# panagiotou23/model-predictive-control

Measured on AMD Instinct MI355X. Metric: MPC solves/sec, bicycle model N=20 nx=4 nu=2, batch=65536; 1/2/4/8 GPU, higher is better.
Workload: dtype f64

## Files before the change

model_predictive_control_amd/csrc/mpc_api.hip:

```cpp
#include "../../include/mpc_hip.h"
#include "mpc_aux.hpp"
#include "mpc_solo.hpp"
#include "mpc_game.hpp"

#include <algorithm>
#include <chrono>
#include <cmath>
#include <cstdio>
#include <cstring>
#include <condition_variable>
#include <mutex>
#include <string>
#include <thread>
#include <array>
#include <vector>

using namespace mpc;

#define MPC_MAX_GROUPS 8
#define MPC_GRID_MAX_ROWS 1024

static thread_local std::string g_err;
static int fail(int code, const std::string &msg) { g_err = msg; return code; }

// ... 242 lines not shown
    int check = 0;
    num(getenv("MPC_CHECK_EVERY"), check);
    if (check > 0) h->check_every = check;
    h->spin = getenv("MPC_SPIN") != nullptr;
    h->host_timing = getenv("MPC_HOST_TIMING") != nullptr;
    if (const char *e = getenv("MPC_HOST_TRACE")) h->host_trace = e;
    const char *hwq = getenv("MPC_HW_QUEUES");
    h->hw_queues = hwq ? atoi(hwq) : probe_stream_concurrency(h);
}

extern "C" int mpc_create(const mpc_config *cfg, int device, mpc_handle **out)
{
    if (!cfg || !out) return fail(MPC_E_ARG, "mpc_create: null argument");
    {
        DevCfg probe;
        const int rcv = make_devcfg(*cfg, probe);
        if (rcv) return rcv;
    }
    int ndev = 0;
    HIPCHK(hipGetDeviceCount(&ndev));
    if (device < 0 || device >= ndev) return fail(MPC_E_ARG, "mpc_create: no such device");
    mpc_handle *h = new mpc_handle();
    h->solo_max = cfg->model == MPC_MODEL_PACEJKA ? 128 : 1024;
    h->solo_all = (cfg->model == MPC_MODEL_KINEMATIC && cfg->N <= 32) ? 4096 : 1024;
    h->cfg = *cfg;
    int rc = make_devcfg(*cfg, h->dc);
    if (rc) { delete h; return rc; }
    h->device = device;
    hipError_t e = hipSetDevice(device);
    if (e == hipSuccess) {
        int cus = 0;
        if (hipDeviceGetAttribute(&cus, hipDeviceAttributeMultiprocessorCount, device) == hipSuccess && cus > 0) h->num_cus = cus;
    }
    if (e == hipSuccess) e = hipHostMalloc((void **)&h->host_counts, 512, hipHostMallocDefault);
    if (e != hipSuccess) { delete h; return fail(MPC_E_HIP, std::string("mpc_create: ") + hipGetErrorString(e)); }
    read_switches(h);
    *out = h;
    return MPC_OK;
}

extern "C" int mpc_destroy(mpc_handle *h)
{
    if (!h) return MPC_OK;
    if (h->worker.joinable()) {
        { std::lock_guard<std::mutex> lk(h->mu); h->worker_quit = true; }
        h->cv.notify_all();
        h->worker.join();
    }
    (void)hipSetDevice(h->device);
    if (h->arena) (void)hipFree(h->arena);
    if (h->stage) (void)hipFree(h->stage);
    if (h->cl_gmeta) (void)hipFree(h->cl_gmeta);
    if (h->cl_gxy) (void)hipFree(h->cl_gxy);
    if (h->cl_gcells) (void)hipFree(h->cl_gcells);
    if (h->host_counts) (void)hipHostFree(h->host_counts);
    if (h->syncev) (void)hipEventDestroy(h->syncev);
    for (auto ev : h->ev_pool) (void)hipEventDestroy(ev);
    for (int g = 0; g < MPC_MAX_GROUPS; g++) if (h->gstream[g]) (void)hipStreamDestroy(h->gstream[g]);
    for (int g = 0; g <= MPC_MAX_GROUPS; g++) if (h->gevent[g]) (void)hipEventDestroy(h->gevent[g]);
    for (int b = 0; b < 2; b++) for (int g = 0; g < MPC_MAX_GROUPS; g++) if (h->pollev[b][g]) (void)hipEventDestroy(h->pollev[b][g]);
    for (int b = 0; b < 2; b++) for (int g = 0; g < MPC_MAX_GROUPS; g++) if (h->soloev[g][b]) (void)hipEventDestroy(h->soloev[g][b]);
    delete h;
    return MPC_OK;
}

static int reserve(mpc_handle *h, int B)
{
    const DevCfg &c = h->dc;
    const int Bp = (B + 63) & ~63;
    if (Bp <= h->Bp_alloc) { h->ws.Bp = h->Bp_alloc; h->ws.B = B; return MPC_OK; }
    HIPCHK(hipSetDevice(h->device));
    if (h->arena) { HIPCHK(hipFree(h->arena)); h->arena = nullptr; h->Bp_alloc = 0; }
    const size_t n = c.n, m = c.m ? c.m : 1, M = c.M, nx = c.nx, N = c.N;
    const size_t JS = nx * (nx + 1) + 2, St = 2 * (size_t)Bp + 64 * (MPC_MAX_GROUPS + 1);
    const size_t nd = 8 * n + 2 * M * n + 7 * m + REC;
    const size_t nscr = (N + 1) * nx + 2 * N + N + N * JS;
    const size_t ni = 4;
    const size_t bytes = (nd * 8 + ni * 4) * (size_t)Bp + nscr * 8 * St + 4 * St + 8 * 4 * MPC_MAX_GROUPS + 256 + 64 + 256;
    char *base = nullptr;
    hipError_t e = hipMalloc((void **)&base, bytes);
    if (e != hipSuccess) return fail(MPC_E_ALLOC, "workspace hipMalloc failed: " + std::string(hipGetErrorString(e)));
    h->arena = base; h->arena_bytes = bytes; h->Bp_alloc = Bp;
    Workspace &w = h->ws;
    double *dp = (double *)base;
    auto takeD = [&](size_t cnt) { double *r = dp; dp += cnt * (size_t)Bp; return r; };
    w.xk = takeD(n); w.gk = takeD(n); w.q = takeD(n); w.xn = takeD(n); w.xe = takeD(n); w.ge = takeD(n);
    w.xe2 = takeD(n); w.ge2 = takeD(n);
    w.S = takeD(M * n); w.Y = takeD(M * n);
    w.Sig = takeD(m); w.Sig_old = takeD(m); w.e1 = takeD(m); w.e2 = takeD(m);
    w.yhx = takeD(m); w.yhxn = takeD(m); w.yhe = takeD(m);
    w.rec = takeD(REC);
    auto takeS = [&](size_t cnt) { double *r = dp; dp += cnt * St; return r; };
    w.trajx = takeS((N + 1) * nx); w.useq = takeS(2 * N); w.stage_L = takeS(N); w.jac = takeS(N * JS);
    int *ip = (int *)dp;
    auto takeI = [&](size_t cnt) { int *r = ip; ip += cnt * (size_t)Bp; return r; };
    w.lists = takeI(4);
    w.agent_of = ip; ip += St;
    w.counts = ip;
    w.totals = (unsigned long long *)(ip + 8 * MPC_MAX_GROUPS);
    w.solo_ctr = (int *)(w.totals + 16);
    w.Bp = Bp; w.B = B; w.St = (int)St; w.Ls = Bp;
    w.ws_xe = w.xe; w.ws_ge = w.ge; w.ws_yhe = w.yhe; w.ws_Sig = w.Sig;
    HIPCHK(hipMemset(base, 0, bytes));
    return MPC_OK;
}

static int reserve_stage(mpc_handle *h, size_t bytes)
{
    if (bytes <= h->stage_bytes) return MPC_OK;
    if (h->stage) { HIPCHK(hipFree(h->stage)); h->stage = nullptr; h->stage_bytes = 0; }
    hipError_t e = hipMalloc((void **)&h->stage, bytes);
    if (e != hipSuccess) return fail(MPC_E_ALLOC, "staging hipMalloc failed");
    h->stage_bytes = bytes;
    return MPC_OK;
}

static inline dim3 grid_for(int B, int block) { return dim3((unsigned)((B + block - 1) / block)); }

template <int MODEL>
static bool launch_eval_t(mpc_handle *h, const Workspace &w, hipStream_t s, const int *lists, const int *counts,
                          int nG, int nC, hipEvent_t eva = nullptr, hipEvent_t evb = nullptr, int slot_bound = -1,
                          int *desc = nullptr)
{
    const DevCfg &c = h->dc;
    const bool shared = w.cl_index == nullptr;
    int nblk = counts ? 2 * (w.Bp / 64) : ((nG + 63) / 64 + (nC + 63) / 64);
    if (counts && slot_bound >= 0) nblk = std::min(nblk, (slot_bound + 126) / 64 + 1);
    if (nblk == 0) return true;
    const size_t lds = sizeof(double) * 64 * (size_t)(c.n + 1) + 64 * sizeof(int);
    bool wide = false;
    if constexpr (MODEL == KIN) {
        wide = counts && slot_bound >= 0 && slot_bound <= h->wide_max && c.nfe == 4 && c.N <= 64;
        if (wide)
            hipLaunchKernelGGL(rollout_wide_kernel, dim3((unsigned)(nblk * 16)), dim3(256), 0, s, c, w, lists, counts);
    }
    bool quad = false;
    if constexpr (MODEL == KIN) {
        quad = !wide && h->quad_rollout && c.nfe == 4 && c.N <= 64;
        if (quad)
            hipLaunchKernelGGL(rollout_pair_kernel, dim3((unsigned)(nblk * 2)), dim3(64),
                               sizeof(double) * 32 * (size_t)(c.n + 1), s, c, w, lists, counts, nG, nC);
    }
    if constexpr (MODEL == PAC) {
        quad = h->quad_rollout && !(counts && slot_bound >= 0 && slot_bound > h->pac_quad_max);
        if (quad)
            hipLaunchKernelGGL(rollout_quad_kernel, dim3((unsigned)(nblk * 4)), dim3(64),
                               sizeof(double) * 16 * (size_t)(c.n + 1), s, c, w, lists, counts, nG, nC);
    }
    if (!wide && !quad)
        hipLaunchKernelGGL((rollout_kernel<MODEL>), dim3((unsigned)nblk), dim3(64), lds, s, c, w, lists, counts, nG, nC);
    if (eva) (void)hipEventRecord(eva, s);
    if constexpr (MODEL == KIN) {
        if (h->fused_eval && (!counts || (slot_bound >= 0 && slot_bound <= h->fused_max))) {
            constexpr int JS = JacRec<MODEL>::SIZE;
            const int spb = FUSED_BLK / c.N;
            const int gb = (nblk * 64 + spb - 1) / spb;
            const size_t flds = sizeof(double) * (size_t)(JS + 1) * c.N * spb;
            if (shared)
                hipLaunchKernelGGL((stage_adjoint_kernel<MODEL, true>), dim3((unsigned)gb), dim3(FUSED_BLK), flds, s, c, w, counts, nG, nC, desc);
            else
                hipLaunchKernelGGL((stage_adjoint_kernel<MODEL, false>), dim3((unsigned)gb), dim3(FUSED_BLK), flds, s, c, w, counts, nG, nC, desc);
            if (evb) (void)hipEventRecord(evb, s);
            return true;
        }
    }
    const size_t xy_lds = (shared && w.near.gmeta && c.S <= GRID_LDS_MAX_S) ? sizeof(double) * 2 * (size_t)c.S : 0;
    if (shared)
        hipLaunchKernelGGL((stage_kernel<MODEL, true>), dim3((unsigned)(nblk * c.N)), dim3(64), xy_lds, s, c, w, counts, nG, nC, nblk);
    else
        hipLaunchKernelGGL((stage_kernel<MODEL, false>), dim3((unsigned)(nblk * c.N)), dim3(64), 0, s, c, w, counts, nG, nC, nblk);
    if (evb) (void)hipEventRecord(evb, s);
    hipLaunchKernelGGL((adjoint_kernel<MODEL>), dim3((unsigned)nblk), dim3(64), 0, s, c, w, counts, nG, nC, desc);
    return false;
}
static bool launch_eval(mpc_handle *h, const Workspace &w, hipStream_t s, const int *lists, const int *counts,
                        int nG, int nC, hipEvent_t eva = nullptr, hipEvent_t evb = nullptr, int slot_bound = -1,
                        int *desc = nullptr)
{
    if (h->dc.model == PAC) return launch_eval_t<PAC>(h, w, s, lists, counts, nG, nC, eva, evb, slot_bound, desc);
    return launch_eval_t<KIN>(h, w, s, lists, counts, nG, nC, eva, evb, slot_bound, desc);
}

static int refuse_if_busy(mpc_handle *h, const char *who)
{
    std::lock_guard<std::mutex> lk(h->mu);
    if (h->job_posted || h->job_running || h->job_done)
        return fail(MPC_E_ARG, std::string(who) + ": a solve of this handle is in flight (mpc_solve_wait first)");
    return MPC_OK;
}
static int check_common(mpc_handle *h, int B, const char *who, bool from_worker = false)
{
    if (!h) return fail(MPC_E_ARG, std::string(who) + ": null handle");
    if (B < 0) return fail(MPC_E_ARG, std::string(who) + ": negative batch");
    if (!from_worker) { const int rb = refuse_if_busy(h, who); if (rb) return rb; }
    HIPCHK(hipSetDevice(h->device));
    return MPC_OK;
}

static NearTab near_for(const mpc_handle *h, const double *cl)
{
    NearTab nt = {nullptr, nullptr, nullptr};
    if (h->nearest_mode == 2 && h->cl_grid_for && h->cl_grid_for == cl) { nt.gmeta = h->cl_gmeta; nt.gcells = h->cl_gcells; nt.gxy = h->cl_gxy; }
    return nt;
}

extern "C" int mpc_centerline_blocks(mpc_handle *h, const double *cl, int C, void *stream)
{
    int rc = check_common(h, C, "mpc_centerline_blocks"); if (rc) return rc;
    h->cl_grid_for = nullptr;
    if (C == 0 || !cl || C > MPC_GRID_MAX_ROWS) return MPC_OK;
    const DevCfg &c = h->dc;
    if (C > h->cl_grid_cap) {
        if (h->cl_gmeta) { HIPCHK(hipFree(h->cl_gmeta)); h->cl_gmeta = nullptr; }
        if (h->cl_gxy) { HIPCHK(hipFree(h->cl_gxy)); h->cl_gxy = nullptr; }
        if (h->cl_gcells) { HIPCHK(hipFree(h->cl_gcells)); h->cl_gcells = nullptr; }
        h->cl_grid_cap = 0;
        if (hipMalloc((void **)&h->cl_gmeta, sizeof(double) * GRID_META * (size_t)C) != hipSuccess ||
            hipMalloc((void **)&h->cl_gxy, sizeof(double) * 2 * (size_t)c.S * (size_t)C) != hipSuccess ||
            hipMalloc((void **)&h->cl_gcells, sizeof(unsigned) * (size_t)GRID_CELLS * (size_t)C) != hipSuccess)
            return fail(MPC_E_ALLOC, "centerline grid hipMalloc failed");
        h->cl_grid_cap = C;
    }
    hipStream_t s = (hipStream_t)stream;
    hipLaunchKernelGGL(cl_grid_meta_kernel, dim3((unsigned)C), dim3(64), 0, s, c, cl, C, h->cl_gmeta, h->cl_gxy);
    hipLaunchKernelGGL(cl_grid_cells_kernel, dim3(GRID_CELLS / 256, C), dim3(256), 0, s, c, cl, C, h->cl_gmeta, h->cl_gcells);
    HIPCHK(hipGetLastError());
    h->cl_grid_for = cl;
    return MPC_OK;
}

extern "C" int mpc_rhs(mpc_handle *h, int B, const double *x, const double *u, double *dx, void *stream)
{
    int rc = check_common(h, B, "mpc_rhs"); if (rc) return rc;
    if (B == 0) return MPC_OK;
    if (!x || !u || !dx) return fail(MPC_E_ARG, "mpc_rhs: null buffer");
    hipStream_t s = (hipStream_t)stream;
    if (h->dc.model == PAC) hipLaunchKernelGGL(rhs_kernel<PAC>, grid_for(B, 64), dim3(64), 0, s, h->dc, B, x, u, dx);
    else hipLaunchKernelGGL(rhs_kernel<KIN>, grid_for(B, 64), dim3(64), 0, s, h->dc, B, x, u, dx);
    HIPCHK(hipGetLastError());
    return MPC_OK;
}

extern "C" int mpc_rollout(mpc_handle *h, int B, int Nsim, const double *x0, const double *U, double *X,
                           void *stream)
{
    int rc = check_common(h, B, "mpc_rollout"); if (rc) return rc;
    if (B == 0 || Nsim == 0) return MPC_OK;
    if (Nsim < 0 || !x0 || !U || !X) return fail(MPC_E_ARG, "mpc_rollout: bad argument");
    hipStream_t s = (hipStream_t)stream;
    if (h->dc.model == PAC) hipLaunchKernelGGL(simulate_kernel<PAC>, grid_for(B, 64), dim3(64), 0, s, h->dc, B, Nsim, x0, U, X);
    else hipLaunchKernelGGL(simulate_kernel<KIN>, grid_for(B, 64), dim3(64), 0, s, h->dc, B, Nsim, x0, U, X);
    HIPCHK(hipGetLastError());
    return MPC_OK;
}

extern "C" int mpc_stage_errors(mpc_handle *h, int B, const double *pose, const double *cl,
                                const int32_t *cl_index, double *err, int32_t *idx, void *stream)
{
    int rc = check_common(h, B, "mpc_stage_errors"); if (rc) return rc;
    if (B == 0) return MPC_OK;
    if (!pose || !cl || !err) return fail(MPC_E_ARG, "mpc_stage_errors: null buffer");
    hipLaunchKernelGGL(errors_kernel, grid_for(B, 64), dim3(64), 0, (hipStream_t)stream, h->dc, B, pose, cl,
                       cl_index, near_for(h, cl), err, idx);
    HIPCHK(hipGetLastError());
    return MPC_OK;
}

extern "C" int mpc_lane_payoff(mpc_handle *h, int B, int K, const double *params15, const double *ego,
                               const double *cars, const int32_t *ncars, double *out, void *stream)
{
    int rc = check_common(h, B, "mpc_lane_payoff"); if (rc) return rc;
    if (B == 0) return MPC_OK;
    if (K < 0 || K > 62 || !params15 || !ego || (K > 0 && !cars) || !ncars || !out)
        return fail(MPC_E_ARG, "mpc_lane_payoff: bad argument");
    LaneParams p;
    std::memcpy(&p, params15, sizeof p);
    hipLaunchKernelGGL(lane_payoff_kernel, grid_for(B, 64), dim3(64), 0, (hipStream_t)stream, p, B, K, ego, cars,
                       ncars, out);
    HIPCHK(hipGetLastError());
    return MPC_OK;
}

extern "C" int mpc_math_probe(mpc_handle *h, int n, int op, const double *a, const double *b, double *out,
                              void *stream)
{
    int rc = check_common(h, n, "mpc_math_probe"); if (rc) return rc;
    if (n == 0) return MPC_OK;
    if (!a || !out || (op == 3 && !b)) return fail(MPC_E_ARG, "mpc_math_probe: null buffer");
    hipLaunchKernelGGL(math_probe_kernel, grid_for(n, 256), dim3(256), 0, (hipStream_t)stream, n, op, a, b, out);
    HIPCHK(hipGetLastError());
    return MPC_OK;
}

extern "C" int mpc_stage_cost(mpc_handle *h, int B, const double *x, const double *u, const double *cl,
                              const int32_t *cl_index, double *out, void *stream)
{
    int rc = check_common(h, B, "mpc_stage_cost"); if (rc) return rc;
    if (B == 0) return MPC_OK;
    if (!x || !u || !cl || !out) return fail(MPC_E_ARG, "mpc_stage_cost: null buffer");
    hipStream_t s = (hipStream_t)stream;
    if (h->dc.model == PAC) hipLaunchKernelGGL(stage_cost_kernel<PAC>, grid_for(B, 64), dim3(64), 0, s, h->dc, B, x, u, cl, cl_index, out);
    else hipLaunchKernelGGL(stage_cost_kernel<KIN>, grid_for(B, 64), dim3(64), 0, s, h->dc, B, x, u, cl, cl_index, out);
    HIPCHK(hipGetLastError());
    return MPC_OK;
}

static int eval_cost_grad(mpc_handle *h, int B, const double *x0, const double *cl, const int32_t *cl_index,
                          const double *U, const double *y, const double *Sigma, double *psi, double *grad,
                          double *yhat, void *stream, bool wave_path);
extern "C" int mpc_eval_cost_grad(mpc_handle *h, int B, const double *x0, const double *cl,
// ... 791 lines not shown
```

model_predictive_control_amd/csrc/mpc_eval.hpp:

```cpp
#pragma once
#include "mpc_solver.hpp"

#ifndef MPC_K1B_WAVES_PAC
#define MPC_K1B_WAVES_PAC 1
#endif
#ifndef MPC_QUAD_WAVES
#define MPC_QUAD_WAVES 2
#endif

namespace mpc {

struct SlotMap {
    int nG, nC, gpad, nblk_g, nblk;
    __device__ SlotMap(const int *counts, int nG_imm, int nC_imm)
    {
        nG = counts ? counts[0] : nG_imm;
        nC = counts ? counts[1] : nC_imm;
        gpad = (nG + 63) & ~63;
        nblk_g = gpad >> 6;
        nblk = nblk_g + ((nC + 63) >> 6);
    }
};

template <int MODEL>
__global__ void __launch_bounds__(64, 2)
rollout_kernel(const DevCfg c, const Workspace w, const int *__restrict__ lists,
               const int *__restrict__ counts, int nG_imm, int nC_imm)
{
    constexpr int NX = ModelDim<MODEL>::NX;
    extern __shared__ double lds[];
    double *tile = lds;
    int *s_agent = (int *)(lds + 64 * (c.n + 1));
    const SlotMap sm(counts, nG_imm, nC_imm);
    const int sb = blockIdx.x;
    if (sb >= sm.nblk) return;
    const int lane = threadIdx.x;
    const bool is_g = sb < sm.nblk_g;
    const int uslot = sb * 64 + lane;
    const int kslot = is_g ? uslot : uslot - sm.gpad;
    const bool active = kslot < (is_g ? sm.nG : sm.nC);
    const int *list = counts ? (is_g ? lists : lists + w.Ls) : nullptr;
    const int raw = active ? (list ? list[kslot] : kslot) : -1;
    const int a = raw < 0 ? -1 : raw & AGENT_MASK;
    const int n = c.n, N = c.N, ld = n + 1;
    s_agent[lane] = raw;
    w.agent_of[uslot] = raw;
    __syncthreads();
    const int total = 64 * n;
    for (int base = 0; base < total; base += 64 * 8) {
        double v[8];
        int off[8];
#pragma unroll
        for (int u = 0; u < 8; u++) {
            const int idx = base + u * 64 + lane;
            const int r = idx / n, j = idx - r * n;
            const int ar = idx < total ? s_agent[r] : -1;
            off[u] = ar >= 0 ? r * ld + j : -1;
            v[u] = ar >= 0 ? ((ar & CH2_BIT) ? w.xe2 : w.xe)[(size_t)(ar & AGENT_MASK) * n + j] : 0.0;
        }
#pragma unroll
        for (int u = 0; u < 8; u++) if (off[u] >= 0) tile[off[u]] = v[u];
    }
    __syncthreads();
    if (!active) return;
    const size_t St = (size_t)w.St;
    const double *urow = tile + lane * ld;
    double x[NX];
#pragma unroll
    for (int i = 0; i < NX; i++) { x[i] = w.x0[(size_t)a * NX + i]; w.trajx[(size_t)i * St + uslot] = x[i]; }
    for (int k = 0; k < N; k++) {
        const double d = urow[2 * k], dl = urow[2 * k + 1];
        w.useq[(size_t)(2 * k) * St + uslot] = d;
        w.useq[(size_t)(2 * k + 1) * St + uslot] = dl;
        StageInput<MODEL> u;
        prep_input(c, d, dl, u);
        stage_forward<MODEL>(c, u, x);
#pragma unroll
        for (int i = 0; i < NX; i++) w.trajx[(size_t)((k + 1) * NX + i) * St + uslot] = x[i];
    }
}

#ifndef MPC_K1A_WAVES
#define MPC_K1A_WAVES 3
#endif
template <class Put>
__device__ __forceinline__ void kin_wide_rollout(const DevCfg &c, const double (&x0)[4], double d, double dl, int lane, Put put);
__global__ void __launch_bounds__(64, MPC_K1A_WAVES)
rollout_pair_kernel(const DevCfg c, const Workspace w, const int *__restrict__ lists,
                    const int *__restrict__ counts, int nG_imm, int nC_imm)
{
#pragma clang fp contract(off)
#if MPC_DEV_STAMP == 1
    DevStamp stamp(blockIdx.x);
#endif
    constexpr int RPB = 32;
    extern __shared__ double lds[];
    const SlotMap sm(counts, nG_imm, nC_imm);
    const int lane = threadIdx.x, q = lane >> 1, half = lane & 1;
    const int uslot = blockIdx.x * RPB + q;
    const int nslots = sm.nblk * 64;
    const bool is_g = uslot < sm.gpad;
    const int kslot = is_g ? uslot : uslot - sm.gpad;
    const bool active = uslot < nslots && kslot < (is_g ? sm.nG : sm.nC);
    const int *list = counts ? (is_g ? lists : lists + w.Ls) : nullptr;
    const int raw = active ? (list ? list[kslot] : kslot) : -1;
    const int n = c.n, N = c.N, ld = n + 1;
    if (half == 0 && uslot < nslots) w.agent_of[uslot] = raw;
    if (__ballot(active) == 0ull) return;
    {
        const double *__restrict__ row = ((raw & CH2_BIT) ? w.xe2 : w.xe) + (size_t)(raw & AGENT_MASK) * n;
        for (int j0 = half; j0 < n; j0 += 16) {
            double v[8];
#pragma unroll
            for (int t = 0; t < 8; t++) v[t] = active && j0 + 2 * t < n ? row[j0 + 2 * t] : 0.0;
#pragma unroll
            for (int t = 0; t < 8; t++) if (j0 + 2 * t < n) lds[q * ld + j0 + 2 * t] = v[t];
        }
    }
    __builtin_amdgcn_wave_barrier();
    const int a = active ? raw & AGENT_MASK : 0;
    const size_t St = (size_t)w.St;
    const double *urow = lds + q * ld;
    double x[4];
#pragma unroll
    for (int i = 0; i < 4; i++) x[i] = active ? w.x0[(size_t)a * 4 + i] : 0.0;
    bool redo = false;
    auto put = [&](int k) {
        if (!active || redo) return;
        w.trajx[(size_t)(k * 4 + 2 * half) * St + uslot] = half ? x[2] : x[0];
        w.trajx[(size_t)(k * 4 + 2 * half + 1) * St + uslot] = half ? x[3] : x[1];
    };
    put(0);
    auto stage = [&](int k, const StageInput<KIN> &u) {
        const double d = urow[2 * k], dl = urow[2 * k + 1];
        if (active) w.useq[(size_t)(2 * k + half) * St + uslot] = half ? dl : d;
        redo = redo || !kin4_in_range(c, u, x);
#if MPC_DEV_STAMP == 1
        if (__ballot(redo) != 0ull) stamp.nfall++;
#endif
        double ph = x[2], v = x[3];
        KinRK k0, k1, k2, k3;
        const double ph0 = ph; kin_rk(c, u, v, k0); kin_next(c, k0, ph, v);
        const double ph1 = ph; kin_rk(c, u, v, k1); kin_next(c, k1, ph, v);
        const double ph2 = ph; kin_rk(c, u, v, k2); kin_next(c, k2, ph, v);
        const double ph3 = ph; kin_rk(c, u, v, k3); kin_next(c, k3, ph, v);
        KinRK ka, kb;
        ka.v1 = half ? k2.v1 : k0.v1; ka.v2 = half ? k2.v2 : k0.v2; ka.v3 = half ? k2.v3 : k0.v3; ka.v4 = half ? k2.v4 : k0.v4;
        ka.kp1 = half ? k2.kp1 : k0.kp1; ka.kp2 = half ? k2.kp2 : k0.kp2; ka.kp3 = half ? k2.kp3 : k0.kp3;
        kb.v1 = half ? k3.v1 : k1.v1; kb.v2 = half ? k3.v2 : k1.v2; kb.v3 = half ? k3.v3 : k1.v3; kb.v4 = half ? k3.v4 : k1.v4;
        kb.kp1 = half ? k3.kp1 : k1.kp1; kb.kp2 = half ? k3.kp2 : k1.kp2; kb.kp3 = half ? k3.kp3 : k1.kp3;
        double dxa, dya, dxb, dyb;
        kin_increment(c, u, half ? ph2 : ph0, ka, !redo, dxa, dya);
        kin_increment(c, u, half ? ph3 : ph1, kb, !redo, dxb, dyb);
        const double oxa = dpp_xchg<0xB1>(dxa), oya = dpp_xchg<0xB1>(dya);
        const double oxb = dpp_xchg<0xB1>(dxb), oyb = dpp_xchg<0xB1>(dyb);
        double px = x[0], py = x[1];
        px = px + dxa; py = py + dya;
        px = px + dxb; py = py + dyb;
        px = px + oxa; py = py + oya;
        px = px + oxb; py = py + oyb;
        x[0] = px; x[1] = py; x[2] = ph; x[3] = v;
        put(k + 1);
    };
    for (int k = 0; k < N; k += 2) {
        const int km = min(k + half, N - 1);
        StageInput<KIN> um, up;
#if MPC_DEV_STAMP == 1
        if (__ballot(!(fabs(urow[2 * km + 1]) <= 0.75)) != 0ull) stamp.nmid++;
        if (__ballot(!(fabs(urow[2 * km + 1]) < 1.0e5)) != 0ull) stamp.nslow++;
#endif
        prep_input(c, urow[2 * km], urow[2 * km + 1], um);
        up.ad = dpp_xchg<0xB1>(um.ad); up.beta = dpp_xchg<0xB1>(um.beta);
        up.sb_lr = dpp_xchg<0xB1>(um.sb_lr); up.cb_lr = dpp_xchg<0xB1>(um.cb_lr);
        up.dbeta = dpp_xchg<0xB1>(um.dbeta); up.mk0 = dpp_xchg<0xB1>(um.mk0); up.mk1 = dpp_xchg<0xB1>(um.mk1);
        StageInput<KIN> ua, ub;
        ua.ad = half ? up.ad : um.ad; ua.beta = half ? up.beta : um.beta; ua.sb_lr = half ? up.sb_lr : um.sb_lr;
        ua.cb_lr = half ? up.cb_lr : um.cb_lr; ua.dbeta = half ? up.dbeta : um.dbeta;
        ua.mk0 = half ? up.mk0 : um.mk0; ua.mk1 = half ? up.mk1 : um.mk1;
        ub.ad = half ? um.ad : up.ad; ub.beta = half ? um.beta : up.beta; ub.sb_lr = half ? um.sb_lr : up.sb_lr;
        ub.cb_lr = half ? um.cb_lr : up.cb_lr; ub.dbeta = half ? um.dbeta : up.dbeta;
        ub.mk0 = half ? um.mk0 : up.mk0; ub.mk1 = half ? um.mk1 : up.mk1;
        stage(k, ua);
        if (k + 1 < N) stage(k + 1, ub);
    }
    unsigned long long todo = __ballot(redo && active && half == 0);
    while (todo != 0ull) {
        const int l0 = (int)__builtin_ctzll(todo);
        todo &= todo - 1ull;
        const int aq = __builtin_amdgcn_readlane(raw, l0) & AGENT_MASK;
        const int uq = blockIdx.x * RPB + (l0 >> 1);
        const double *uro = lds + (l0 >> 1) * ld;
        const bool stage_lane = lane < N;
        const double dq = stage_lane ? uro[2 * lane] : 0.0, dlq = stage_lane ? uro[2 * lane + 1] : 0.0;
        double xq[4];
#pragma unroll
        for (int i = 0; i < 4; i++) xq[i] = w.x0[(size_t)aq * 4 + i];
        double *const tj = w.trajx + uq;
        kin_wide_rollout(c, xq, dq, dlq, lane, [=](int k, int i, double v) { tj[(size_t)(k * 4 + i) * St] = v; });
    }
}


__global__ void __launch_bounds__(64, MPC_QUAD_WAVES)
rollout_quad_kernel(const DevCfg c, const Workspace w, const int *__restrict__ lists,
                    const int *__restrict__ counts, int nG_imm, int nC_imm)
{
    constexpr int NX = 6, RPB = 16;
    extern __shared__ double lds[];
#if MPC_DEV_STAMP == 4
    DevStamp stamp(blockIdx.x);
#endif
    const SlotMap sm(counts, nG_imm, nC_imm);
    const int lane = threadIdx.x, q = lane >> 2, role = lane & 3;
    const int uslot = blockIdx.x * RPB + q;
    const int nslots = sm.nblk * 64;
    const bool is_g = uslot < sm.gpad;
    const int kslot = is_g ? uslot : uslot - sm.gpad;
    const bool active = uslot < nslots && kslot < (is_g ? sm.nG : sm.nC);
    const int *list = counts ? (is_g ? lists : lists + w.Ls) : nullptr;
    const int raw = active ? (list ? list[kslot] : kslot) : -1;
    const int n = c.n, N = c.N, ld = n + 1;
    if (role == 0 && uslot < nslots) w.agent_of[uslot] = raw;
    if (active) {
        const double *__restrict__ row = ((raw & CH2_BIT) ? w.xe2 : w.xe) + (size_t)(raw & AGENT_MASK) * n;
        for (int j0 = role; j0 < n; j0 += 32) {
            double v[8];
#pragma unroll
            for (int t = 0; t < 8; t++) v[t] = j0 + 4 * t < n ? row[j0 + 4 * t] : 0.0;
#pragma unroll
            for (int t = 0; t < 8; t++) if (j0 + 4 * t < n) lds[q * ld + j0 + 4 * t] = v[t];
        }
    }
    __builtin_amdgcn_wave_barrier();
    if (!active) return;
    const int a = raw & AGENT_MASK;
    const size_t St = (size_t)w.St;
    const double *urow = lds + q * ld;
    double x[NX];
#pragma unroll
    for (int i = 0; i < NX; i++) x[i] = w.x0[(size_t)a * NX + i];
    auto put = [&](int k) {
        w.trajx[(size_t)(k * NX + role) * St + uslot] = role == 0 ? x[0] : role == 1 ? x[1] : role == 2 ? x[2] : x[3];
        if (role < 2) w.trajx[(size_t)(k * NX + 4 + role) * St + uslot] = role == 0 ? x[4] : x[5];
    };
    put(0);
    for (int k = 0; k < N; k++) {
        const double d = urow[2 * k], dl = urow[2 * k + 1];
        if (role == 0) w.useq[(size_t)(2 * k) * St + uslot] = d;
        if (role == 1) w.useq[(size_t)(2 * k + 1) * St + uslot] = dl;
        StageInput<PAC> u;
        prep_input(c, d, dl, u);
#if MPC_DEV_STAMP == 4
        {
            bool fin = true;
#pragma unroll
            for (int i = 0; i < NX; i++) fin = fin && fabs(x[i]) < 1.0e300;
            const bool inr = fabs(x[2]) < 1.0e5 && fabs(dl) < 1.0e5 && (x[3] != 0.0 || (x[5] * c.lf + x[4] != 0.0 && x[5] * c.lr - x[4] != 0.0));
            if (__ballot(!fin) != 0ull) stamp.nfall++;
            if (__ballot(fin && !inr) != 0ull) stamp.nmid++;
            if (__ballot(!fin) != 0ull && k == 0) stamp.nslow++;
        }
#endif
        stage_forward_quad(c, u, x, role);
        put(k + 1);
    }
}

template <class Put>
__device__ __forceinline__ void kin_wide_rollout(const DevCfg &c, const double (&x0)[4], double d, double dl, int lane, Put put)
{
    const int N = c.N;
    const bool stage_lane = lane < N;
    StageInput<KIN> u;
    prep_input(c, d, dl, u);
    if (lane == 0) {
#pragma unroll
        for (int i = 0; i < 4; i++) put(0, i, x0[i]);
    }
    double ph = x0[2], v = x0[3];
    constexpr int PASS = 4;
    double cph[PASS] = {0.0, 0.0, 0.0, 0.0}, cv[PASS] = {0.0, 0.0, 0.0, 0.0}, eph = 0.0, ev = 0.0;
    int gen = 0;
    bool anygen = false;
#pragma unroll
    for (int p = 0; p < PASS; p++) {
        const int k1 = N < 16 * (p + 1) ? N : 16 * (p + 1);
        for (int k = 16 * p; k < k1; k++) {
            StageInput<KIN> uk;
            uk.ad = rdlane(u.ad, k); uk.beta = rdlane(u.beta, k); uk.sb_lr = rdlane(u.sb_lr, k);
            const double xs[4] = {0.0, 0.0, ph, v};
            const bool inr = __ballot(!kin4_in_range(c, uk, xs)) == 0ull;
            anygen = anygen || !inr;
#pragma unroll
            for (int j = 0; j < 4; j++) {
                if (lane == ((4 * k + j) & 63)) { cph[p] = ph; cv[p] = v; gen |= inr ? 0 : 1 << p; }
                KinRK kr;
                if (inr) { kin_rk(c, uk, v, kr); kin_next(c, kr, ph, v); }
                else { kin_gen_rk(c, uk, v, kr); kin_gen_next(c, kr, ph, v); }
            }
            if (lane == k) { eph = ph; ev = v; }
        }
    }
    double dx[PASS] = {0.0, 0.0, 0.0, 0.0}, dy[PASS] = {0.0, 0.0, 0.0, 0.0};
#pragma unroll
    for (int p = 0; p < PASS; p++) {
        const int s = 64 * p + lane;
        if (64 * p >= 4 * N) break;
        const int k = (s >> 2) < N ? (s >> 2) : N - 1;
        StageInput<KIN> uk;
        uk.ad = __shfl(u.ad, k); uk.beta = __shfl(u.beta, k); uk.sb_lr = __shfl(u.sb_lr, k);
        const bool g = ((gen >> p) & 1) != 0 && (s >> 2) < N;
        KinRK kr;
        kin_rk(c, uk, cv[p], kr);
        kin_increment(c, uk, cph[p], kr, !g, dx[p], dy[p]);
        if (anygen) {
            double gx, gy;
            kin_gen_rk(c, uk, g ? cv[p] : 0.0, kr);
            kin_gen_increment(c, uk, g ? cph[p] : 0.0, g ? cv[p] : 0.0, kr, gx, gy);
            dx[p] = g ? gx : dx[p]; dy[p] = g ? gy : dy[p];
        }
    }
    double px = x0[0], py = x0[1], epx = 0.0, epy = 0.0;
#pragma unroll
    for (int p = 0; p < PASS; p++) {
        const int k0 = 16 * p, k1 = N < 16 * (p + 1) ? N : 16 * (p + 1);
        for (int k = k0; k < k1; k++) {
#pragma clang fp contract(off)
#pragma unroll
            for (int j = 0; j < 4; j++) {
                px = px + rdlane(dx[p], (4 * k + j) & 63);
                py = py + rdlane(dy[p], (4 * k + j) & 63);
            }
            if (lane == k) { epx = px; epy = py; }
        }
    }
    if (stage_lane) { put(lane + 1, 0, epx); put(lane + 1, 1, epy); put(lane + 1, 2, eph); put(lane + 1, 3, ev); }
}

__global__ void __launch_bounds__(256)
rollout_wide_kernel(const DevCfg c, const Workspace w, const int *__restrict__ lists,
                    const int *__restrict__ counts)
{
    const SlotMap sm(counts, 0, 0);
    const int lane = threadIdx.x & 63, wv = threadIdx.x >> 6;
    const int uslot = blockIdx.x * 4 + wv;
    if (uslot >= sm.nblk * 64) return;
    const bool is_g = uslot < sm.gpad;
    const int kslot = is_g ? uslot : uslot - sm.gpad;
    const bool active = kslot < (is_g ? sm.nG : sm.nC);
    const int raw = active ? (is_g ? lists : lists + w.Ls)[kslot] : -1;
    if (lane == 0) w.agent_of[uslot] = raw;
    if (!active) return;
    const int a = raw & AGENT_MASK;
    const int N = c.N, n = c.n;
    const size_t St = (size_t)w.St;
    const double *__restrict__ row = ((raw & CH2_BIT) ? w.xe2 : w.xe) + (size_t)a * n;
    const bool stage_lane = lane < N;
    const double d = stage_lane ? row[2 * lane] : 0.0, dl = stage_lane ? row[2 * lane + 1] : 0.0;
    if (stage_lane) {
        w.useq[(size_t)(2 * lane) * St + uslot] = d;
        w.useq[(size_t)(2 * lane + 1) * St + uslot] = dl;
    }
    double x0[4];
#pragma unroll
    for (int i = 0; i < 4; i++) x0[i] = w.x0[(size_t)a * 4 + i];
    double *const tj = w.trajx + uslot;
    kin_wide_rollout(c, x0, d, dl, lane,
                     [=](int k, int i, double v) { tj[(size_t)(k * 4 + i) * St] = v; });
}

template <int MODEL> struct JacRec { static constexpr int SIZE = ModelDim<MODEL>::NX * (ModelDim<MODEL>::NX + 1) + 2; };

__device__ __forceinline__ void stage_geom(const DevCfg &c, const Workspace &w, const double *__restrict__ clp, int row,
                                           double px, double py, Geom &g)
{
    load_geom(c, clp, nearest_lookup(c, clp, w.near, row, px, py), g);
}

template <int MODEL, class Put>
__device__ __forceinline__ void stage_record(const DevCfg &c, const Workspace &w, int a, bool ch2, bool is_g,
                                             int k, const double (&xs)[ModelDim<MODEL>::NX],
                                             const double (&xe)[ModelDim<MODEL>::NX], double d, double dl,
                                             const Geom &g, Put put)
{
    constexpr int NX = ModelDim<MODEL>::NX, JS = JacRec<MODEL>::SIZE;
    double xb[NX], ub[2] = {0.0, 0.0};
#pragma unroll
    for (int i = 0; i < NX; i++) xb[i] = 0.0;
    double L = is_g ? stage_cost<MODEL, true>(c, g, xe, d, dl, xb, ub)
                    : stage_cost<MODEL, false>(c, g, xe, d, dl, xb, ub);
    if (c.sm) {
#pragma clang fp contract(off)
        const size_t am = (size_t)a * c.m;
#pragma unroll
        for (int i = 0; i < NX; i++) {
            if (i < c.sm) {
                const size_t kk = am + (size_t)(k * c.sm + i);
                const double gv = stage_constraint<MODEL>(c, g, xe, i);
                double lb, ubd;
                constraint_bounds(c, i, lb, ubd);
                const double sg = w.Sig[kk];
                const double zeta = gv + w.y[kk] / sg;
                const double zhat = fmax(lb, fmin(zeta, ubd));
                const double dd = zeta - zhat;
                const double yh = sg * dd;
                L = fma(0.5 * dd, yh, L);
                if (!ch2) w.yhe[kk] = yh;
                if (is_g) stage_constraint_adjoint<MODEL>(c, g, xe, i, yh, xb);
            }
        }
    }
    put(JS, L);
    if (is_g) {
#pragma unroll
        for (int i = 0; i < NX; i++) put(i, xb[i]);
        put(NX, ub[0]);
        put(NX + 1, ub[1]);
    }
}

template <int MODEL> __device__ __forceinline__ constexpr bool sens_is_const(int dd, int i)
{
    return (dd == 0 && i >= 2) || (MODEL == KIN && dd == 3 && i == 3);
}
__device__ __forceinline__ constexpr double sens_const(int dd, int i) { return dd == 0 && i == 2 ? 1.0 : 0.0; }

template <int MODEL, class Put>
__device__ __forceinline__ void stage_sens_record(const DevCfg &c, const double (&xs)[ModelDim<MODEL>::NX],
                                                  const double (&xe)[ModelDim<MODEL>::NX], double d, double dl, Put put)
{
    constexpr int NX = ModelDim<MODEL>::NX;
    StageInput<MODEL> u;
    prep_input(c, d, dl, u);
    double T[NX][NX];
    if constexpr (MODEL == PAC) {
        const bool lost = pac_stage_is_lost(u, xs);
        double xp[NX];
#pragma unroll
        for (int i = 0; i < NX; i++) xp[i] = xs[i];
        if (lost) pac_park(u, xp);
        stage_tangents_at<MODEL>(c, u, xp, xe, T);
#pragma unroll
        for (int dd = 0; dd < NX; dd++) {
#pragma unroll
            for (int i = 0; i < NX; i++)
                if (!sens_is_const<MODEL>(dd, i)) put(NX + 2 + dd * NX + i, lost ? __builtin_nan("") : T[dd][i]);
        }
        return;
    }
    stage_tangents_at<MODEL>(c, u, xs, xe, T);
#pragma unroll
    for (int dd = 0; dd < NX; dd++) {
#pragma unroll
        for (int i = 0; i < NX; i++) if (!sens_is_const<MODEL>(dd, i)) put(NX + 2 + dd * NX + i, T[dd][i]);
    }
}

template <int MODEL, class Get>
__device__ __forceinline__ void adjoint_rec_to(const DevCfg &c, bool is_g, Get get, double *psi_out, double *grow)
{
    constexpr int NX = ModelDim<MODEL>::NX, NZ = NX - 2, JS = JacRec<MODEL>::SIZE;
    const int N = c.N;
    double psi = 0.0;
    for (int k = 0; k < N; k++) psi += get(k, JS);
    if (psi_out) *psi_out = psi;
    if (!is_g) return;
    double lam[NX];
#pragma unroll
    for (int i = 0; i < NX; i++) lam[i] = 0.0;
    for (int k = N - 1; k >= 0; k--) {
#pragma unroll
        for (int i = 0; i < NX; i++) lam[i] += get(k, i);
        double gu[2], lz[NZ];
#pragma unroll
        for (int jj = 0; jj < 2; jj++) {
            double acc = get(k, NX + jj);
#pragma unroll
            for (int i = 0; i < NX; i++)
                acc = fma(sens_is_const<MODEL>(NZ + jj, i) ? sens_const(NZ + jj, i) : get(k, NX + 2 + (NZ + jj) * NX + i), lam[i], acc);
            gu[jj] = acc;
        }
#pragma unroll
        for (int jj = 0; jj < NZ; jj++) {
            double acc = 0.0;
#pragma unroll
            for (int i = 0; i < NX; i++)
                acc = fma(sens_is_const<MODEL>(jj, i) ? sens_const(jj, i) : get(k, NX + 2 + jj * NX + i), lam[i], acc);
            lz[jj] = acc;
        }
#pragma unroll
        for (int jj = 0; jj < NZ; jj++) lam[2 + jj] = lz[jj];
        grow[2 * k] = gu[0];
        grow[2 * k + 1] = gu[1];
    }
}
template <int MODEL, class Get>
__device__ __forceinline__ void adjoint_rec(const DevCfg &c, const Workspace &w, int a, bool ch2, bool is_g, Get get)
{
    double *psi_out = w.psi_direct ? w.psi_direct + a : !ch2 ? w.rec + (size_t)a * REC + R_PSIE : nullptr;
    adjoint_rec_to<MODEL>(c, is_g, get, psi_out, (ch2 ? w.ge2 : w.ge) + (size_t)a * c.n);
}

template <class Get>
__device__ __forceinline__ void adjoint_rec_quad_kin(const DevCfg &c, bool is_g, int comp, Get get, double *psi_out, double *grow)
{
    constexpr int NX = 4, NZ = 2, JS = JacRec<KIN>::SIZE;
    const int N = c.N;
    if (comp == 0) {
        double psi = 0.0;
        for (int k = 0; k < N; k++) psi += get(k, JS);
        if (psi_out) *psi_out = psi;
    }
    if (!is_g) return;
    const int dd = (comp + 2) & 3;
    double lam = 0.0;
    for (int k = N - 1; k >= 0; k--) {
        lam += get(k, comp);
        const double l0 = quad_bcast<0x00>(lam), l1 = quad_bcast<0x55>(lam), l2 = quad_bcast<0xAA>(lam), l3 = quad_bcast<0xFF>(lam);
        double acc = comp < 2 ? get(k, NX + comp) : 0.0;
        const double t0 = get(k, NX + 2 + dd * NX + 0), t1 = get(k, NX + 2 + dd * NX + 1);
        const double t2 = dd == 0 ? 1.0 : get(k, NX + 2 + dd * NX + 2);
        const double t3 = (dd == 0 || dd == 3) ? 0.0 : get(k, NX + 2 + dd * NX + 3);
        acc = fma(t0, l0, acc);
        acc = fma(t1, l1, acc);
        acc = fma(t2, l2, acc);
        acc = fma(t3, l3, acc);
        if (comp < 2) grow[2 * k + comp] = acc;
        else lam = acc;
    }
    static_assert(sens_is_const<KIN>(0, 2) && sens_is_const<KIN>(0, 3) && sens_is_const<KIN>(3, 3) && !sens_is_const<KIN>(3, 2) &&
                  !sens_is_const<KIN>(1, 3) && !sens_is_const<KIN>(2, 3) && !sens_is_const<KIN>(0, 1), "constant entries of the kinematic block");
    (void)NZ;
}

#ifndef MPC_K1B_WAVES
#define MPC_K1B_WAVES 3
#endif

template <int MODEL, bool SHARED_CL>
__global__ void __launch_bounds__(64, (MODEL == KIN ? MPC_K1B_WAVES : MPC_K1B_WAVES_PAC))
stage_kernel(const DevCfg c, const Workspace w, const int *__restrict__ counts, int nG_imm, int nC_imm,
             int nblk_max)
{
    constexpr int NX = ModelDim<MODEL>::NX, JS = JacRec<MODEL>::SIZE;
#if MPC_DEV_STAMP == 6
    DevStamp stamp(blockIdx.x);
#endif
    const SlotMap sm(counts, nG_imm, nC_imm);
    const int k = blockIdx.x / nblk_max, sb = blockIdx.x % nblk_max;
    if (sb >= sm.nblk) return;
    const bool is_g = sb < sm.nblk_g;
    const int uslot = sb * 64 + threadIdx.x;
    const int raw = w.agent_of[uslot];
    extern __shared__ double2 s_xy[];
    const bool lds_xy = SHARED_CL && w.near.gmeta != nullptr && c.S <= GRID_LDS_MAX_S;
    if (lds_xy) {
        const double2 *__restrict__ gp = reinterpret_cast<const double2 *>(w.near.gxy);
        for (int j = threadIdx.x; j < c.S; j += 64) s_xy[j] = gp[j];
        __builtin_amdgcn_wave_barrier();
    }
    if (raw < 0) return;
    const int a = raw & AGENT_MASK;
    const bool ch2 = (raw & CH2_BIT) != 0;
    const size_t St = (size_t)w.St;
    double xs[NX], xe[NX];
#pragma unroll
    for (int i = 0; i < NX; i++) {
        xs[i] = w.trajx[(size_t)(k * NX + i) * St + uslot];
        xe[i] = w.trajx[(size_t)((k + 1) * NX + i) * St + uslot];
    }
    const double d = w.useq[(size_t)(2 * k) * St + uslot], dl = w.useq[(size_t)(2 * k + 1) * St + uslot];
    const double *__restrict__ clp = SHARED_CL ? w.cl : w.cl + (size_t)w.cl_index[a] * 2 * (size_t)c.S;
    double *const jr = w.jac + (size_t)k * JS * St + uslot;
    double *const sl = w.stage_L + (size_t)k * St + uslot;
    const auto put = [=](int f, double v) { *(f == JS ? sl : jr + (size_t)f * St) = v; };
    if (is_g) stage_sens_record<MODEL>(c, xs, xe, d, dl, put);
    Geom g;
    if (lds_xy) {
        const int idx = nearest_index_grid(c, clp, w.near.gmeta, w.near.gcells, [=](int i) { return s_xy[i]; }, xe[0], xe[1]);
        load_geom_xy(s_xy, idx, g);
    } else {
        stage_geom(c, w, clp, SHARED_CL ? 0 : w.cl_index[a], xe[0], xe[1], g);
    }
    stage_record<MODEL>(c, w, a, ch2, is_g, k, xs, xe, d, dl, g, put);
}

template <int MODEL>
__global__ void __launch_bounds__(64)
adjoint_kernel(const DevCfg c, const Workspace w, const int *__restrict__ counts, int nG_imm, int nC_imm,
               int *__restrict__ desc)
{
    constexpr int JS = JacRec<MODEL>::SIZE;
    const SlotMap sm(counts, nG_imm, nC_imm);
    const int sb = blockIdx.x;
    if (desc && sb == 0 && threadIdx.x == 0) *desc = sm.gpad;
    if (sb >= sm.nblk) return;
    const bool is_g = sb < sm.nblk_g;
    const int uslot = sb * 64 + threadIdx.x;
    const int raw = w.agent_of[uslot];
    if (raw < 0) return;
    const size_t St = (size_t)w.St;
    const double *const jac = w.jac + uslot, *const sl = w.stage_L + uslot;
    adjoint_rec<MODEL>(c, w, raw & AGENT_MASK, (raw & CH2_BIT) != 0, is_g, [=](int k, int f) {
        return f == JS ? sl[(size_t)k * St] : jac[((size_t)k * JS + f) * St];
    });
}

constexpr int FUSED_BLK = 256;

#ifndef MPC_FUSED_WAVES
#define MPC_FUSED_WAVES 3
#endif
template <int MODEL, bool SHARED_CL>
__global__ void __launch_bounds__(FUSED_BLK, MPC_FUSED_WAVES)
stage_adjoint_kernel(const DevCfg c, const Workspace w, const int *__restrict__ counts, int nG_imm, int nC_imm,
                     int *__restrict__ desc)
{
    static_assert(MODEL == KIN, "the fused K1b + K1c kernel is the kinematic model's");
    constexpr int NX = ModelDim<MODEL>::NX, JS = JacRec<MODEL>::SIZE, BLK = FUSED_BLK;
    extern __shared__ double s_rec[];
#if MPC_DEV_STAMP == 2
    DevStamp stamp(blockIdx.x * (BLK / 64) + (threadIdx.x >> 6));
#endif
    const SlotMap sm(counts, nG_imm, nC_imm);
    const int N = c.N, SPB = BLK / N;
    const int slot0 = blockIdx.x * SPB, nslots = sm.nblk * 64;
    if (desc && blockIdx.x == 0 && threadIdx.x == 0) *desc = sm.gpad;
    if (slot0 >= nslots) return;
    const size_t St = (size_t)w.St;
    const int NS = N * SPB;
    {
        const int k = threadIdx.x / SPB, j = threadIdx.x - k * SPB;
        const int uslot = slot0 + j;
        const int raw = (k < N && uslot < nslots) ? w.agent_of[uslot] : -1;
        if (raw >= 0) {
            const bool is_g = uslot < sm.gpad;
            const int a = raw & AGENT_MASK;
            const bool ch2 = (raw & CH2_BIT) != 0;
            double xs[NX], xe[NX];
#pragma unroll
            for (int i = 0; i < NX; i++) {
                xs[i] = w.trajx[(size_t)(k * NX + i) * St + uslot];
                xe[i] = w.trajx[(size_t)((k + 1) * NX + i) * St + uslot];
            }
            const double d = w.useq[(size_t)(2 * k) * St + uslot], dl = w.useq[(size_t)(2 * k + 1) * St + uslot];
            const double *__restrict__ clp = SHARED_CL ? w.cl : w.cl + (size_t)w.cl_index[a] * 2 * (size_t)c.S;
            double *const r = s_rec + k * SPB + j;
            const auto put = [=](int f, double v) { r[(size_t)f * NS] = v; };
            if (is_g) stage_sens_record<MODEL>(c, xs, xe, d, dl, put);
            Geom g;
            stage_geom(c, w, clp, SHARED_CL ? 0 : w.cl_index[a], xe[0], xe[1], g);
            stage_record<MODEL>(c, w, a, ch2, is_g, k, xs, xe, d, dl, g, put);
        }
    }
    __syncthreads();
    for (int t = threadIdx.x; t < 4 * SPB; t += BLK) {
        const int j = t >> 2, comp = t & 3, uslot = slot0 + j;
        const int raw = uslot < nslots ? w.agent_of[uslot] : -1;
        if (raw < 0) continue;
        const double *const rj = s_rec + j;
        const int a = raw & AGENT_MASK;
        const bool ch2 = (raw & CH2_BIT) != 0;
        double *psi_out = w.psi_direct ? w.psi_direct + a : !ch2 ? w.rec + (size_t)a * REC + R_PSIE : nullptr;
        adjoint_rec_quad_kin(c, uslot < sm.gpad, comp, [=](int k, int f) { return rj[(size_t)f * NS + k * SPB]; },
                             psi_out, (ch2 ? w.ge2 : w.ge) + (size_t)a * c.n);
    }
}

}
```

Before: 501,400.

## Split kinematic sensitivity into hot/cold paths and compact fused LDS record

Adds a hot path for the kinematic stage sensitivities that uses the endpoint-aware RK4 tangent routine when inputs are in range. Out-of-range lanes fall back to a cold path that reloads the state and recomputes the tangents after a ballot. The fused stage-adjoint kernel's shared-memory record drops three constant rows through a row remap, which shrinks LDS per block. Kernel arguments are re-fetched through a KernArgs accessor inside scoped blocks, apparently to shorten register live ranges. The cost is more code and a divergent cold path, and the compact row mapping must stay in sync with the adjoint reader.

```diff
diff --git a/model_predictive_control_amd/csrc/mpc_api.hip b/model_predictive_control_amd/csrc/mpc_api.hip
--- a/model_predictive_control_amd/csrc/mpc_api.hip
+++ b/model_predictive_control_amd/csrc/mpc_api.hip
@@ -418,10 +418,10 @@
     if (eva) (void)hipEventRecord(eva, s);
     if constexpr (MODEL == KIN) {
         if (h->fused_eval && (!counts || (slot_bound >= 0 && slot_bound <= h->fused_max))) {
-            constexpr int JS = JacRec<MODEL>::SIZE;
-            const int spb = FUSED_BLK / c.N;
+            const FusedTile tile(c.N);
+            const int spb = tile.spb;
             const int gb = (nblk * 64 + spb - 1) / spb;
-            const size_t flds = sizeof(double) * (size_t)(JS + 1) * c.N * spb;
+            const size_t flds = tile.bytes();
             if (shared)
                 hipLaunchKernelGGL((stage_adjoint_kernel<MODEL, true>), dim3((unsigned)gb), dim3(FUSED_BLK), flds, s, c, w, counts, nG, nC, desc);
             else
diff --git a/model_predictive_control_amd/csrc/mpc_eval.hpp b/model_predictive_control_amd/csrc/mpc_eval.hpp
--- a/model_predictive_control_amd/csrc/mpc_eval.hpp
+++ b/model_predictive_control_amd/csrc/mpc_eval.hpp
@@ -86,10 +86,12 @@
 template <class Put>
 __device__ __forceinline__ void kin_wide_rollout(const DevCfg &c, const double (&x0)[4], double d, double dl, int lane, Put put);
 __global__ void __launch_bounds__(64, MPC_K1A_WAVES)
-rollout_pair_kernel(const DevCfg c, const Workspace w, const int *__restrict__ lists,
+rollout_pair_kernel(const DevCfg cfg, const Workspace ws, const int *__restrict__ lists,
                     const int *__restrict__ counts, int nG_imm, int nC_imm)
 {
 #pragma clang fp contract(off)
+    const DevCfg &c = cfg;
+    const Workspace &w = ws;
 #if MPC_DEV_STAMP == 1
     DevStamp stamp(blockIdx.x);
 #endif
@@ -119,21 +121,21 @@
     }
     __builtin_amdgcn_wave_barrier();
     const int a = active ? raw & AGENT_MASK : 0;
-    const size_t St = (size_t)w.St;
     const double *urow = lds + q * ld;
     double x[4];
 #pragma unroll
     for (int i = 0; i < 4; i++) x[i] = active ? w.x0[(size_t)a * 4 + i] : 0.0;
     bool redo = false;
-    auto put = [&](int k) {
+    auto put = [&](const Workspace &w, int k) {
         if (!active || redo) return;
+        const size_t St = (size_t)w.St;
         w.trajx[(size_t)(k * 4 + 2 * half) * St + uslot] = half ? x[2] : x[0];
         w.trajx[(size_t)(k * 4 + 2 * half + 1) * St + uslot] = half ? x[3] : x[1];
     };
-    put(0);
-    auto stage = [&](int k, const StageInput<KIN> &u) {
+    put(w, 0);
+    auto stage = [&](const DevCfg &c, const Workspace &w, int k, const StageInput<KIN> &u) {
         const double d = urow[2 * k], dl = urow[2 * k + 1];
-        if (active) w.useq[(size_t)(2 * k + half) * St + uslot] = half ? dl : d;
+        if (active) w.useq[(size_t)(2 * k + half) * (size_t)w.St + uslot] = half ? dl : d;
         redo = redo || !kin4_in_range(c, u, x);
 #if MPC_DEV_STAMP == 1
         if (__ballot(redo) != 0ull) stamp.nfall++;
@@ -160,9 +162,12 @@
         px = px + oxa; py = py + oya;
         px = px + oxb; py = py + oyb;
         x[0] = px; x[1] = py; x[2] = ph; x[3] = v;
-        put(k + 1);
+        put(w, k + 1);
     };
     for (int k = 0; k < N; k += 2) {
+        const KernArgs ka;
+        const DevCfg &c = ka.c();
+        const Workspace &w = ka.w();
         const int km = min(k + half, N - 1);
         StageInput<KIN> um, up;
 #if MPC_DEV_STAMP == 1
@@ -180,11 +185,15 @@
         ub.ad = half ? um.ad : up.ad; ub.beta = half ? um.beta : up.beta; ub.sb_lr = half ? um.sb_lr : up.sb_lr;
         ub.cb_lr = half ? um.cb_lr : up.cb_lr; ub.dbeta = half ? um.dbeta : up.dbeta;
         ub.mk0 = half ? um.mk0 : up.mk0; ub.mk1 = half ? um.mk1 : up.mk1;
-        stage(k, ua);
-        if (k + 1 < N) stage(k + 1, ub);
+        stage(c, w, k, ua);
+        if (k + 1 < N) stage(c, w, k + 1, ub);
     }
     unsigned long long todo = __ballot(redo && active && half == 0);
     while (todo != 0ull) {
+        const KernArgs ka;
+        const DevCfg &c = ka.c();
+        const Workspace &w = ka.w();
+        const size_t St = (size_t)w.St;
         const int l0 = (int)__builtin_ctzll(todo);
         todo &= todo - 1ull;
         const int aq = __builtin_amdgcn_readlane(raw, l0) & AGENT_MASK;
@@ -456,6 +465,41 @@
     }
 }
 
+template <class Put>
+__device__ __forceinline__ bool stage_sens_record_kin_hot(const DevCfg &c, const double (&xs)[4], const double (&xe)[4],
+                                                          double d, double dl, Put put)
+{
+    StageInput<KIN> u;
+    prep_input(c, d, dl, u);
+    const bool ok = c.nfe == 4 && kin4_in_range(c, u, xs);
+    const double xa[4] = {xs[0], xs[1], ok ? xs[2] : 0.0, ok ? xs[3] : 0.0};
+    double T[4][4];
+    stage_tangents_kin4(c, u, xa, xe, T);
+#pragma unroll
+    for (int dd = 0; dd < 4; dd++) {
+#pragma unroll
+        for (int i = 0; i < 4; i++) if (!sens_is_const<KIN>(dd, i)) put(6 + dd * 4 + i, T[dd][i]);
+    }
+    return !ok;
+}
+template <class Put>
+__device__ __forceinline__ void stage_sens_record_kin_cold(const DevCfg &c, const double *__restrict__ trajx,
+                                                           const double *__restrict__ useq, size_t St, Put put)
+{
+    double xs[4];
+#pragma unroll
+    for (int i = 0; i < 4; i++) xs[i] = trajx[(size_t)i * St];
+    StageInput<KIN> u;
+    prep_input(c, useq[0], useq[St], u);
+    double T[4][4];
+    stage_tangents<KIN>(c, u, xs, T);
+#pragma unroll
+    for (int dd = 0; dd < 4; dd++) {
+#pragma unroll
+        for (int i = 0; i < 4; i++) if (!sens_is_const<KIN>(dd, i)) put(6 + dd * 4 + i, T[dd][i]);
+    }
+}
+
 template <int MODEL, class Get>
 __device__ __forceinline__ void adjoint_rec_to(const DevCfg &c, bool is_g, Get get, double *psi_out, double *grow)
 {
@@ -574,7 +618,11 @@
     double *const jr = w.jac + (size_t)k * JS * St + uslot;
     double *const sl = w.stage_L + (size_t)k * St + uslot;
     const auto put = [=](int f, double v) { *(f == JS ? sl : jr + (size_t)f * St) = v; };
-    if (is_g) stage_sens_record<MODEL>(c, xs, xe, d, dl, put);
+    bool cold = false;
+    if (is_g) {
+        if constexpr (MODEL == KIN) cold = stage_sens_record_kin_hot(c, xs, xe, d, dl, put);
+        else stage_sens_record<MODEL>(c, xs, xe, d, dl, put);
+    }
     Geom g;
     if (lds_xy) {
         const int idx = nearest_index_grid(c, clp, w.near.gmeta, w.near.gcells, [=](int i) { return s_xy[i]; }, xe[0], xe[1]);
@@ -583,6 +631,14 @@
         stage_geom(c, w, clp, SHARED_CL ? 0 : w.cl_index[a], xe[0], xe[1], g);
     }
     stage_record<MODEL>(c, w, a, ch2, is_g, k, xs, xe, d, dl, g, put);
+    if constexpr (MODEL == KIN) {
+        if (__builtin_expect(__ballot(cold) != 0ull, 0)) {
+            const KernArgs ka;
+            const Workspace &wc = ka.w();
+            const size_t Sc = (size_t)wc.St;
+            if (cold) stage_sens_record_kin_cold(ka.c(), wc.trajx + (size_t)(k * NX) * Sc + uslot, wc.useq + (size_t)(2 * k) * Sc + uslot, Sc, put);
+        }
+    }
 }
 
 template <int MODEL>
@@ -607,13 +663,22 @@
 }
 
 constexpr int FUSED_BLK = 256;
+struct FusedTile {
+    static constexpr int ROWS = JacRec<KIN>::SIZE + 1 - 3;
+    int spb, ns;
+    __host__ __device__ explicit FusedTile(int N) : spb(FUSED_BLK / N), ns(N * (FUSED_BLK / N)) {}
+    __host__ __device__ size_t bytes() const { return sizeof(double) * (size_t)ROWS * ns; }
+    __host__ __device__ static constexpr int row(int f) { return f == JacRec<KIN>::SIZE ? ROWS - 1 : f >= 6 + 4 ? f - 2 : f; }
+};
+static_assert(FusedTile::row(6 + 1) == 7 && FusedTile::row(6 + 4) == 8 && FusedTile::row(6 + 14) == 18 &&
+              FusedTile::row(JacRec<KIN>::SIZE) == 19 && FusedTile::ROWS == 20, "the rows of the kinematic record");
 
 #ifndef MPC_FUSED_WAVES
 #define MPC_FUSED_WAVES 3
 #endif
 template <int MODEL, bool SHARED_CL>
 __global__ void __launch_bounds__(FUSED_BLK, MPC_FUSED_WAVES)
-stage_adjoint_kernel(const DevCfg c, const Workspace w, const int *__restrict__ counts, int nG_imm, int nC_imm,
+stage_adjoint_kernel(const DevCfg cfg, const Workspace ws, const int *__restrict__ counts, int nG_imm, int nC_imm,
                      int *__restrict__ desc)
 {
     static_assert(MODEL == KIN, "the fused K1b + K1c kernel is the kinematic model's");
@@ -622,38 +687,69 @@
 #if MPC_DEV_STAMP == 2
     DevStamp stamp(blockIdx.x * (BLK / 64) + (threadIdx.x >> 6));
 #endif
-    const SlotMap sm(counts, nG_imm, nC_imm);
-    const int N = c.N, SPB = BLK / N;
+    int nG, nC, N;
+    {
+        const SlotMap sm0(counts, nG_imm, nC_imm);
+        nG = sm0.nG; nC = sm0.nC; N = cfg.N;
+        (void)ws;
+    }
+    const SlotMap sm(nullptr, nG, nC);
+    const FusedTile tile(N);
+    const int SPB = tile.spb, NS = tile.ns;
     const int slot0 = blockIdx.x * SPB, nslots = sm.nblk * 64;
     if (desc && blockIdx.x == 0 && threadIdx.x == 0) *desc = sm.gpad;
     if (slot0 >= nslots) return;
-    const size_t St = (size_t)w.St;
-    const int NS = N * SPB;
     {
         const int k = threadIdx.x / SPB, j = threadIdx.x - k * SPB;
         const int uslot = slot0 + j;
-        const int raw = (k < N && uslot < nslots) ? w.agent_of[uslot] : -1;
+        bool cold = false;
+        double *const r = s_rec + k * SPB + j;
+        const auto put = [=](int f, double v) { r[(size_t)FusedTile::row(f) * NS] = v; };
+        int raw;
+        {
+            const KernArgs ka;
+            raw = (k < N && uslot < nslots) ? ka.w().agent_of[uslot] : -1;
+        }
         if (raw >= 0) {
             const bool is_g = uslot < sm.gpad;
             const int a = raw & AGENT_MASK;
             const bool ch2 = (raw & CH2_BIT) != 0;
-            double xs[NX], xe[NX];
-#pragma unroll
-            for (int i = 0; i < NX; i++) {
-                xs[i] = w.trajx[(size_t)(k * NX + i) * St + uslot];
-                xe[i] = w.trajx[(size_t)((k + 1) * NX + i) * St + uslot];
+            double xs[NX], xe[NX], d, dl;
+            {
+                const KernArgs ka;
+                const DevCfg &c = ka.c();
+                const Workspace &w = ka.w();
+                const size_t St = (size_t)w.St;
+#pragma unroll
+                for (int i = 0; i < NX; i++) {
+                    xs[i] = w.trajx[(size_t)(k * NX + i) * St + uslot];
+                    xe[i] = w.trajx[(size_t)((k + 1) * NX + i) * St + uslot];
+                }
+                d = w.useq[(size_t)(2 * k) * St + uslot]; dl = w.useq[(size_t)(2 * k + 1) * St + uslot];
+                if (is_g) cold = stage_sens_record_kin_hot(c, xs, xe, d, dl, put);
             }
-            const double d = w.useq[(size_t)(2 * k) * St + uslot], dl = w.useq[(size_t)(2 * k + 1) * St + uslot];
-            const double *__restrict__ clp = SHARED_CL ? w.cl : w.cl + (size_t)w.cl_index[a] * 2 * (size_t)c.S;
-            double *const r = s_rec + k * SPB + j;
-            const auto put = [=](int f, double v) { r[(size_t)f * NS] = v; };
-            if (is_g) stage_sens_record<MODEL>(c, xs, xe, d, dl, put);
-            Geom g;
-            stage_geom(c, w, clp, SHARED_CL ? 0 : w.cl_index[a], xe[0], xe[1], g);
-            stage_record<MODEL>(c, w, a, ch2, is_g, k, xs, xe, d, dl, g, put);
+            {
+                const KernArgs ka;
+                const DevCfg &c = ka.c();
+                const Workspace &w = ka.w();
+                const int row = SHARED_CL ? 0 : w.cl_index[a];
+                const double *__restrict__ clp = w.cl + (size_t)row * 2 * (size_t)c.S;
+                Geom g;
+                stage_geom(c, w, clp, row, xe[0], xe[1], g);
+                stage_record<MODEL>(c, w, a, ch2, is_g, k, xs, xe, d, dl, g, put);
+            }
+        }
+        if (__builtin_expect(__ballot(cold) != 0ull, 0)) {
+            const KernArgs ka;
+            const Workspace &w = ka.w();
+            const size_t St = (size_t)w.St;
+            if (cold) stage_sens_record_kin_cold(ka.c(), w.trajx + (size_t)(k * NX) * St + uslot, w.useq + (size_t)(2 * k) * St + uslot, St, put);
         }
     }
     __syncthreads();
+    const KernArgs ka;
+    const DevCfg &c = ka.c();
+    const Workspace &w = ka.w();
     for (int t = threadIdx.x; t < 4 * SPB; t += BLK) {
         const int j = t >> 2, comp = t & 3, uslot = slot0 + j;
         const int raw = uslot < nslots ? w.agent_of[uslot] : -1;
@@ -662,9 +758,10 @@
         const int a = raw & AGENT_MASK;
         const bool ch2 = (raw & CH2_BIT) != 0;
         double *psi_out = w.psi_direct ? w.psi_direct + a : !ch2 ? w.rec + (size_t)a * REC + R_PSIE : nullptr;
-        adjoint_rec_quad_kin(c, uslot < sm.gpad, comp, [=](int k, int f) { return rj[(size_t)f * NS + k * SPB]; },
+        adjoint_rec_quad_kin(c, uslot < sm.gpad, comp, [=](int k, int f) { return rj[(size_t)FusedTile::row(f) * NS + k * SPB]; },
                              psi_out, (ch2 ? w.ge2 : w.ge) + (size_t)a * c.n);
     }
-}
-
-}
+    (void)JS;
+}
+
+}
```

New measurement: 499,800 (median of 2 runs). About the same (-0.3%).
